# YichengDWu/tinyedm

Measured on AMD Instinct MI355X. Metric: train imgs/sec CIFAR-10 32x32 bf16, higher is better.
Workload: dtype bf16

## Files before the change

include/tinyedm_hip.h:

```cpp
#ifndef TINYEDM_HIP_H
#define TINYEDM_HIP_H
#ifdef __cplusplus
extern "C" {
#endif

typedef struct ihipStream_t* edm_stream_t;

int edm_version(void);
const char* edm_last_error(void);
int edm_init(int device);
int edm_graph_replay_safe(void);
typedef struct {
  unsigned step, seed_lo, seed_hi, reserved;
  float lr, ema_beta, grad_scale, bc1, bc2sqrt, pad[3];
} edm_step_params;

int edm_conv_igemm(const void* X, const void* Wp, void* Y, const void* R, float alpha, float beta, int B, int H,
                   int W, int Cin, int Cout, int taps, edm_stream_t stream);
int edm_conv_igemm_v2(const void* X, const void* Wp, void* Y, const void* R, float alpha, float beta, int B, int H,
                      int W, int Cin, int Cout, int taps, edm_stream_t stream);
int edm_conv_igemm_v6(const void* X, const void* Wp, void* Y, const void* R, float alpha, float beta, int B, int H,
                      int W, int Cin, int Cout, int taps, edm_stream_t stream);
int edm_conv_igemm_s(const void* X, const void* Wp, void* Y, const void* R, float alpha, float beta, int B, int H,
                     int W, int Cin, int Cout, int taps, edm_stream_t stream);
// ... 103 lines not shown
int edm_dropout_mask(unsigned char* mask, long n, float pdrop, unsigned long long seed, unsigned sub, unsigned step,
                     edm_stream_t stream);
int edm_pool2(const void* x, void* y, int B, int Hout, int Wout, int C, float scale, edm_stream_t stream);
int edm_up2(const void* x, const void* add, void* y, int B, int Hout, int Wout, int C, float scale, edm_stream_t stream);
int edm_up2_silu(const void* x, void* y, void* a, int B, int Hout, int Wout, int C, edm_stream_t stream);
int edm_reduce_hw(const void* x, long x_stride, const void* y, long y_stride, float* out, int B, int HW, int C,
                  float scale, edm_stream_t stream);
int edm_scalelong_fwd(const float* mean, const float* W1h, const float* W2h, float* gate, float* z1save, int B, int C,
                      int R, edm_stream_t stream);
int edm_scalelong_bwd(const float* mean, const float* W1h, const float* W2h, const float* gate, const float* z1save,
                      const float* ggate, float* gmean, float* gW1h, float* gW2h, int B, int C, int R,
                      edm_stream_t stream);
int edm_skip_gate_fwd(const void* skip, const float* W1h, const float* W2h, float* mean, float* gate, float* z1save,
                      int B, int HW, int C, int R, edm_stream_t stream);
int edm_skip_gate_bwd(const void* gcat, long gcat_stride, int c_off, const void* skip, const float* mean,
                      const float* W1h, const float* W2h, const float* gate, const float* z1save, float* gmean,
                      float* gW1h, float* gW2h, float* ws, int B, int HW, int C, int R, edm_stream_t stream);
typedef struct {
  const float* ws;
  const float* mean;
  float* gW1h;
  float* gW2h;
  int B, C, R, pad;
} edm_skip_gate_wgrad_item;
long edm_skip_gate_wgrad_multi_table_bytes(void);
int edm_skip_gate_wgrad_multi(const edm_skip_gate_wgrad_item* items, int n, void* table_host, void* table_dev,
                              int defer_upload, edm_stream_t stream);
typedef struct {
  const void* skip;
  const float* W1h;
  const float* W2h;
  float* mean;
  float* gate;
  float* z1save;
  void* cat;
  void* silu_out;
  int B, HW, C, R, Ci, pad;
} edm_skip_gate_fwd_item;
long edm_skip_gate_fwd_multi_table_bytes(void);
int edm_skip_gate_fwd_multi(const edm_skip_gate_fwd_item* items, int n, void* table_host, void* table_dev, int defer_upload,
                            edm_stream_t stream);
typedef struct {
  const void* gcat;
  long gcat_stride;
  const void* skip;
  const float* W1h;
  const float* W2h;
  const float* gate;
  const float* z1save;
  float* gmean;
  float* ws;
  void* gskip;
  int c_off, B, HW, C, R, pad;
} edm_skip_gate_bwd_item;
typedef struct {
  const void* gcs;
  const float* gate;
  const float* gmean;
  void* gskip;
  int B, HW, Cs, pad;
} edm_skip_half_bwd_item;
long edm_skip_gate_bwd_multi_table_bytes(void);
int edm_skip_gate_bwd_multi(const edm_skip_gate_bwd_item* items, int n, void* table_host, void* table_dev, int defer_upload,
                            edm_stream_t stream);
int edm_skip_half_bwd_multi(const edm_skip_half_bwd_item* items, int n, void* table_host, void* table_dev, int defer_upload,
                            edm_stream_t stream);
int edm_concat_gate_fwd(const void* inp, const void* skip, const float* gate, void* cat, void* silu_out, int B, int HW,
                        int Ci, int Cs, edm_stream_t stream);
int edm_concat_gate_bwd(const void* gcat, const float* gate, const float* gmean, void* ginp, void* gskip, int B,
                        int HW, int Ci, int Cs, edm_stream_t stream);
int edm_skip_half_fwd(const void* skip, const float* gate, void* cat, void* silu_out, int B, int HW, int Ci, int Cs,
                      edm_stream_t stream);
int edm_skip_half_bwd(const void* gcs, const float* gate, const float* gmean, void* gskip, int B, int HW, int Cs,
                      edm_stream_t stream);

int edm_precond_in(const float* noisy, const float* sigma, int sigma_stride, float sigma_data, void* out, int B,
                   int Cimg, int HW, int CP, edm_stream_t stream);
int edm_conv_out_fwd(const void* x, const float* w_hat, const float* gain_out, const float* noisy, const float* sigma,
                     int sigma_stride, float sigma_data, float* D, float* Fraw, int B, int HW, int C, int Co,
                     edm_stream_t stream);
int edm_conv_out_bwd(const void* x, const float* w_hat, const float* gain_out, const float* Fraw, const float* dD,
                     const float* sigma, int sigma_stride, float sigma_data, void* gx, float* gw_hat, float* ggain,
                     int B, int HW, int C, int Co, edm_stream_t stream);
int edm_nchw_to_nhwc_bf16(const float* x, void* y, int B, int C, int HW, edm_stream_t stream);
int edm_nhwc_bf16_to_nchw(const void* x, float* y, int B, int C, int HW, edm_stream_t stream);

int edm_linear_fwd(const float* X, const float* W, float* Y, int M, int N, int K, edm_stream_t stream);
int edm_linear_dgrad(const float* dY, const float* W, float* dX, int M, int N, int K, int accumulate,
                     edm_stream_t stream);
int edm_linear_wgrad(const float* dY, const float* X, float* dW, int M, int N, int K, int accumulate,
                     edm_stream_t stream);
int edm_fourier_fwd(const float* sigma, int sigma_stride, const float* freqs, const float* phases, float* out, int B,
                    int Fd, edm_stream_t stream);
int edm_embed_combine_fwd(const float* emb_sigma, const float* wcls_hat, const long long* labels, float add_factor,
                          int K, float* pre, float* out, int B, int E, edm_stream_t stream);
int edm_embed_combine_bwd(const float* gout, const float* pre, const long long* labels, float add_factor, int K,
                          float* gemb_sigma, float* gwcls_hat, int B, int E, edm_stream_t stream);

int edm_diffuse(const float* clean, float* noisy, float* sigma, float P_mean, float P_std, int B, long CHW,
                unsigned long long seed, unsigned step, const void* dyn, edm_stream_t stream);
int edm_diffuse_given(const float* clean, const float* eps, const float* noise, float* noisy, float* sigma,
                      float P_mean, float P_std, int B, long CHW, edm_stream_t stream);
int edm_weighted_mse(const float* D, const float* clean, const float* sigma, const float* weight_override,
                     float sigma_data, float* loss, float* dD, int B, long CHW, float* acc_sum, long long* acc_total,
                     edm_stream_t stream);
int edm_adam_ema(float* theta, float* grad, float* m, float* v, float* ema, long n, float lr, float b1, float b2,
                 float eps, int step, float ema_beta, float grad_scale, const void* dyn, int zero_grad,
                 unsigned* health, edm_stream_t stream);
int edm_heun_euler(const float* x, const float* D, float t0, float t1, float* dx, float* x1, long n, unsigned* health,
                   edm_stream_t stream);
int edm_heun_correct(const float* x, const float* dx, const float* x1, const float* D1, float t0, float t1, float* out,
                     long n, unsigned* health, edm_stream_t stream);
int edm_heun_euler_guided(const float* x, const float* Dm, const float* Dg, const float* w, float t0, float t1,
                          float* dx, float* x1, long n, unsigned* health, edm_stream_t stream);
int edm_heun_correct_guided(const float* x, const float* dx, const float* x1, const float* Dm1, const float* Dg1,
                            const float* w, float t0, float t1, float* out, long n, unsigned* health,
                            edm_stream_t stream);
int edm_heun_churn(const float* x, float c, const void* rec, int step, int B, long CHW, float* x_hat,
                   unsigned* health, edm_stream_t stream);
int edm_scale_f32(const float* x, float s, float* y, long n, edm_stream_t stream);

int edm_f32_conv(const float* X, const float* w_hat, float* Y, const float* R, float alpha, float beta, const float* lin,
                 long lin_stride, const float* gain, int B, int H, int W, int Cin, int I, int Cout, int taps,
                 edm_stream_t stream);
int edm_f32_to_pairs(const float* x, void* pairs, long rows, int C, edm_stream_t stream);
int edm_split_pack(const float* w_hat, void* pack, int O, int I, int taps, int Ip, edm_stream_t stream);
int edm_split_conv(const void* Xp, const void* Wp3, float* Y, void* Ypairs, const float* R, float alpha, float beta,
                   const float* lin, long lin_stride, const float* gain, int B, int H, int W, int C, int Cout, int taps,
                   edm_stream_t stream);
int edm_split_conv_o(const void* Xp, const void* Wp3, float* Y, void* Ypairs, long ld_pairs, long lo_off, void* Ysilu_pairs,
                     const float* R, float alpha, float beta, const float* lin, long lin_stride, const float* gain, int B,
                     int H, int W, int C, int Cout, int taps, edm_stream_t stream);
int edm_split_conv_fold(const void* Xp, const void* Wp3, const void* X2p, const void* W2p3, int C2, float* Y, void* Ypairs,
                        long ld_pairs, long lo_off, void* Ysilu_pairs, float alpha3, float alpha1, int B, int H, int W, int C,
                        int Cout, edm_stream_t stream);
int edm_f32_skip_half(const float* skip, const float* gate, void* cat_pairs, void* silu_pairs, int B, int HW, int Ci, int Cs,
                      edm_stream_t stream);
int edm_f32_attention(const float* qkv, float* y, int B, int N, int C, int heads, edm_stream_t stream);
int edm_split_attention(const float* qkv, float* y, void* ypairs, int B, int N, int C, int heads, edm_stream_t stream);
int edm_f32_pixelnorm_silu(const float* x, float* xn, float* s, long P, int C, int s_pairs, edm_stream_t stream);
int edm_f32_silu(const float* x, float* s, long n, int pairs_row, edm_stream_t stream);
int edm_f32_pool2(const float* x, float* y, int B, int Hout, int Wout, int C, edm_stream_t stream);
int edm_f32_up2(const float* x, float* y, int B, int Hout, int Wout, int C, edm_stream_t stream);
int edm_f32_pool_pixelnorm_silu(const float* x, float* xn, float* s, int B, int Hout, int Wout, int C, int s_pairs,
                                edm_stream_t stream);
int edm_f32_up2_silu(const float* x, float* y, float* s, int B, int Hout, int Wout, int C, int s_pairs, edm_stream_t stream);
int edm_f32_skip_gate(const float* skip, const float* W1h, const float* W2h, float* gate, int B, int HW, int C, int R,
                      edm_stream_t stream);
int edm_f32_concat_gate(const float* inp, const float* skip, const float* gate, float* cat, float* silu_out, int B,
                        int HW, int Ci, int Cs, int pairs, edm_stream_t stream);
int edm_f32_precond_in(const float* noisy, const float* sigma, int sigma_stride, float sigma_data, float* out, int B,
                       int Cimg, int HW, int CP, edm_stream_t stream);
int edm_f32_conv_out(const float* x, const float* w_hat, const float* gain_out, const float* noisy, const float* sigma,
                     int sigma_stride, float sigma_data, float* D, int B, int HW, int C, int Co, edm_stream_t stream);
int edm_f32_nchw_to_nhwc(const float* x, float* y, int B, int C, int HW, edm_stream_t stream);
int edm_f32_nhwc_to_nchw(const float* x, float* y, int B, int C, int HW, edm_stream_t stream);

int edm_u8_gather_normalize(const void* data, const long* index, float* out, int B, int C, int H, int W, long n_images,
                            float mean, float stdv, int flip, unsigned long long seed, unsigned epoch,
                            edm_stream_t stream);
int edm_denormalize_u8(const float* x, void* out, long n, float scale, float offset, edm_stream_t stream);
int edm_prediction_to_u8_nhwc(const float* pred, void* out, int B, int C, int H, int W, const float* mean,
                              const float* stdv, edm_stream_t stream);

#ifdef __cplusplus
}
// ... 3 lines not shown
```

tinyedm_amd/_lib.py:

```python
import ctypes
import os

_HERE = os.path.dirname(os.path.abspath(__file__))
LIB_PATH = os.environ.get("EDM_LIB_PATH") or os.path.join(_HERE, "libtinyedm_hip.so")

P, I, L, F = ctypes.c_void_p, ctypes.c_int, ctypes.c_long, ctypes.c_float
U, U64 = ctypes.c_uint, ctypes.c_ulonglong

SIGNATURES = {
    "edm_version": [],
    "edm_last_error": [],
    "edm_init": [I],
    "edm_graph_replay_safe": [],
    "edm_pixelnorm_silu_fwd": [P, P, P, P, L, I, P],
    "edm_pixelnorm_silu_bwd": [P, P, P, F, P, P, P, L, I, P],
    "edm_pool_pixelnorm_silu_fwd": [P, P, P, P, I, I, I, I, P],
    "edm_pool_pixelnorm_silu_bwd": [P, P, P, F, P, P, P, I, I, I, I, P],
    "edm_up2_silu": [P, P, P, I, I, I, I, P],
    "edm_silu_fwd": [P, P, L, P],
    "edm_silu_bwd": [P, P, P, F, P, L, P],
    "edm_axpby": [P, F, P, F, P, L, P],
    "edm_mod_silu_drop_fwd": [P, P, L, P, P, I, I, I, F, U64, U, U, P, P],
    "edm_mod_silu_drop_bwd": [P, P, L, P, P, P, P, P, L, P, I, I, I, F, U64, U, U, P, P],
    "edm_mod_silu_drop_bwd_raw": [P, P, L, P, P, P, P, L, I, I, I, F, U64, U, U, P, P],
    "edm_dropout_mask": [P, L, F, U64, U, U, P],
    "edm_pool2": [P, P, I, I, I, I, F, P],
    "edm_up2": [P, P, P, I, I, I, I, F, P],
    "edm_reduce_hw": [P, L, P, L, P, I, I, I, F, P],
    "edm_scalelong_fwd": [P, P, P, P, P, I, I, I, P],
    "edm_scalelong_bwd": [P, P, P, P, P, P, P, P, P, I, I, I, P],
    "edm_skip_gate_fwd": [P, P, P, P, P, P, I, I, I, I, P],
    "edm_skip_gate_bwd": [P, L, I, P, P, P, P, P, P, P, P, P, P, I, I, I, I, P],
    "edm_skip_gate_wgrad_multi": [P, I, P, P, I, P],
    "edm_skip_gate_wgrad_multi_table_bytes": [],
    "edm_skip_gate_fwd_multi": [P, I, P, P, I, P],
    "edm_skip_gate_fwd_multi_table_bytes": [],
    "edm_skip_gate_bwd_multi": [P, I, P, P, I, P],
    "edm_skip_half_bwd_multi": [P, I, P, P, I, P],
    "edm_skip_gate_bwd_multi_table_bytes": [],
    "edm_concat_gate_fwd": [P, P, P, P, P, I, I, I, I, P],
    "edm_concat_gate_bwd": [P, P, P, P, P, I, I, I, I, P],
    "edm_skip_half_fwd": [P, P, P, P, I, I, I, I, P],
    "edm_skip_half_bwd": [P, P, P, P, I, I, I, P],
    "edm_precond_in": [P, P, I, F, P, I, I, I, I, P],
    "edm_conv_out_fwd": [P, P, P, P, P, I, F, P, P, I, I, I, I, P],
    "edm_conv_out_bwd": [P, P, P, P, P, P, I, F, P, P, P, I, I, I, I, P],
    "edm_nchw_to_nhwc_bf16": [P, P, I, I, I, P],
    "edm_nhwc_bf16_to_nchw": [P, P, I, I, I, P],
    "edm_conv_igemm": [P, P, P, P, F, F, I, I, I, I, I, I, P],
    "edm_conv_igemm_v2": [P, P, P, P, F, F, I, I, I, I, I, I, P],
    "edm_conv_igemm_o": [P, P, P, L, P, P, L, I, P, F, F, I, I, I, I, I, I, I, I, P],
    "edm_conv3x3_fold_supported": [I, I, I, I, I, I],
    "edm_conv3x3_fold": [P, P, P, L, P, I, P, L, P, F, F, I, I, I, I, I, P],
    "edm_conv_igemm_v6": [P, P, P, P, F, F, I, I, I, I, I, I, P],
    "edm_conv_igemm_s": [P, P, P, P, F, F, I, I, I, I, I, I, P],
    "edm_conv3x3_mod": [P, P, P, P, P, L, P, F, U64, U, U, I, I, I, I, I, I, P, I, P],
    "edm_conv3x3_modbwd": [P, P, F, P, P, L, P, P, P, L, F, U64, U, U, I, I, I, I, I, I, P, I, P],
    "edm_mod_finish_multi": [P, P, P, L, P, I, I, P],
    "edm_conv3x3_silubwd": [P, P, P, P, F, P, I, I, I, I, I, I, P],
    "edm_mod_finish": [P, P, L, P, P, L, P, I, I, P],
    "edm_conv_wgrad_nsplit": [I, I, I, I, I, I],
    "edm_conv_wgrad_v2": [P, P, P, I, I, I, I, I, I, I, P],
    "edm_conv_wgrad_1x1_nsplit": [L, I, I],
    "edm_conv_wgrad_1x1_nsplit_grouped": [L, I, I],
    "edm_conv_wgrad_1x1": [P, P, P, L, I, I, I, P],
    "edm_conv_wgrad_1x1_group": [P, I, P, P, I, P],
    "edm_conv_wgrad_1x1_group_table_bytes": [],
    "edm_wgrad3_workspace": [P, I],
    "edm_wgrad3_group": [P, I, P, L, P, P, I, P],
    "edm_wgrad3_table_bytes": [],
    "edm_wgrad3_max_layers": [],
    "edm_attention_fwd": [P, P, I, I, I, I, P],
    "edm_attention_bwd": [P, P, P, P, I, I, I, I, P],
    "edm_attention_qkv_supported": [I, I, I],
    "edm_attention_qkv_fwd": [P, P, P, P, I, I, I, I, I, P],
    "edm_attention_qkv_bwd": [P, P, P, P, P, P, P, F, I, I, I, I, I, P],
    "edm_linear_fwd": [P, P, P, I, I, I, P],
    "edm_linear_dgrad": [P, P, P, I, I, I, I, P],
    "edm_linear_wgrad": [P, P, P, I, I, I, I, P],
    "edm_fourier_fwd": [P, I, P, P, P, I, I, P],
    "edm_embed_combine_fwd": [P, P, P, F, I, P, P, I, I, P],
    "edm_embed_combine_bwd": [P, P, P, F, I, P, P, I, I, P],
    "edm_diffuse": [P, P, P, F, F, I, L, U64, U, P, P],
    "edm_diffuse_given": [P, P, P, P, P, F, F, I, L, P],
    "edm_weighted_mse": [P, P, P, P, F, P, P, I, L, P, P, P],
    "edm_adam_ema": [P, P, P, P, P, L, F, F, F, F, I, F, F, P, I, P, P],
    "edm_heun_euler": [P, P, F, F, P, P, L, P, P],
    "edm_heun_correct": [P, P, P, P, F, F, P, L, P, P],
    "edm_heun_euler_guided": [P, P, P, P, F, F, P, P, L, P, P],
    "edm_heun_correct_guided": [P, P, P, P, P, P, F, F, P, L, P, P],
    "edm_heun_churn": [P, F, P, I, I, L, P, P, P],
    "edm_scale_f32": [P, F, P, L, P],
    "edm_weight_prep": [P, I, I, I, I, P, P, P, P, I, P],
    "edm_weight_prep_multi": [P, P, I, I, I, P],
    "edm_wgrad_finish": [P, I, P, P, P, I, I, I, I, F, I, P],
    "edm_wgrad_finish_multi": [P, I, P, P, I, P],
    "edm_wgrad_finish_multi_table_bytes": [],
    "edm_f32_conv": [P, P, P, P, F, F, P, L, P, I, I, I, I, I, I, I, P],
    "edm_f32_attention": [P, P, I, I, I, I, P],
    "edm_split_attention": [P, P, P, I, I, I, I, P],
    "edm_f32_to_pairs": [P, P, L, I, P],
    "edm_split_pack": [P, P, I, I, I, I, P],
    "edm_split_conv": [P, P, P, P, P, F, F, P, L, P, I, I, I, I, I, I, P],
    "edm_split_conv_o": [P, P, P, P, L, L, P, P, F, F, P, L, P, I, I, I, I, I, I, P],
    "edm_split_conv_fold": [P, P, P, P, I, P, P, L, L, P, F, F, I, I, I, I, I, P],
    "edm_f32_skip_half": [P, P, P, P, I, I, I, I, P],
    "edm_f32_pool_pixelnorm_silu": [P, P, P, I, I, I, I, I, P],
    "edm_f32_up2_silu": [P, P, P, I, I, I, I, I, P],
    "edm_f32_pixelnorm_silu": [P, P, P, L, I, I, P],
    "edm_f32_silu": [P, P, L, I, P],
    "edm_f32_pool2": [P, P, I, I, I, I, P],
    "edm_f32_up2": [P, P, I, I, I, I, P],
    "edm_f32_skip_gate": [P, P, P, P, I, I, I, I, P],
    "edm_f32_concat_gate": [P, P, P, P, P, I, I, I, I, I, P],
    "edm_f32_precond_in": [P, P, I, F, P, I, I, I, I, P],
    "edm_f32_conv_out": [P, P, P, P, P, I, F, P, I, I, I, I, P],
    "edm_f32_nchw_to_nhwc": [P, P, I, I, I, P],
    "edm_f32_nhwc_to_nchw": [P, P, I, I, I, P],
    "edm_u8_gather_normalize": [P, P, P, I, I, I, I, L, F, F, I, U64, U, P],
    "edm_denormalize_u8": [P, P, L, F, F, P],
    "edm_prediction_to_u8_nhwc": [P, P, I, I, I, I, P, P, P],
}
DIAG_SIGNATURES = {
    "edm_conv_igemm_v2_stamp": [P, P, P, I, I, I, I, I, P, P],
    "edm_conv_igemm_v2_ablate": [P, P, P, I, I, I, I, I, I, P],
    "edm_wgrad3_probe": [P, P],
    "edm_wgrad3_plan_ksplit": [P, I, P],
    "edm_v6_persistent_launches": [],
}
_RET = {"edm_last_error": ctypes.c_char_p, "edm_v6_persistent_launches": ctypes.c_long, "edm_wgrad3_workspace": ctypes.c_long, "edm_wgrad3_table_bytes": ctypes.c_long,
        "edm_skip_gate_wgrad_multi_table_bytes": ctypes.c_long, "edm_skip_gate_fwd_multi_table_bytes": ctypes.c_long, "edm_skip_gate_bwd_multi_table_bytes": ctypes.c_long,
        "edm_conv_wgrad_1x1_group_table_bytes": ctypes.c_long, "edm_wgrad_finish_multi_table_bytes": ctypes.c_long}
_NO_STATUS = {"edm_skip_gate_bwd_multi_table_bytes", "edm_skip_gate_fwd_multi_table_bytes", "edm_v6_persistent_launches", "edm_conv3x3_fold_supported", "edm_skip_gate_wgrad_multi_table_bytes", "edm_version", "edm_graph_replay_safe", "edm_last_error", "edm_conv_wgrad_nsplit", "edm_conv_wgrad_1x1_nsplit", "edm_conv_wgrad_1x1_nsplit_grouped", "edm_wgrad3_workspace", "edm_wgrad3_table_bytes", "edm_wgrad3_max_layers",
              "edm_conv_wgrad_1x1_group_table_bytes", "edm_wgrad_finish_multi_table_bytes", "edm_attention_qkv_supported"}

_lib = None


class HipKernelError(RuntimeError):
    pass


class FinishItem(ctypes.Structure):
    _fields_ = [("slabs", P), ("w", P), ("grad", P), ("perm", P), ("S", I), ("O", I), ("I", I), ("Ipad", I), ("taps", I),
                ("scale", F), ("accumulate", I)]


class SkipGateWgradItem(ctypes.Structure):
    _fields_ = [("ws", P), ("mean", P), ("gW1h", P), ("gW2h", P), ("B", I), ("C", I), ("R", I), ("pad", I)]


class SkipGateFwdItem(ctypes.Structure):
    _fields_ = [("skip", P), ("W1h", P), ("W2h", P), ("mean", P), ("gate", P), ("z1save", P), ("cat", P), ("silu_out", P),
                ("B", I), ("HW", I), ("C", I), ("R", I), ("Ci", I), ("pad", I)]


class SkipGateBwdItem(ctypes.Structure):
    _fields_ = [("gcat", P), ("gcat_stride", L), ("skip", P), ("W1h", P), ("W2h", P), ("gate", P), ("z1save", P), ("gmean", P),
                ("ws", P), ("gskip", P), ("c_off", I), ("B", I), ("HW", I), ("C", I), ("R", I), ("pad", I)]


class SkipHalfBwdItem(ctypes.Structure):
    _fields_ = [("gcs", P), ("gate", P), ("gmean", P), ("gskip", P), ("B", I), ("HW", I), ("Cs", I), ("pad", I)]


class WGrad1Item(ctypes.Structure):
    _fields_ = [("X", P), ("dY", P), ("slabs", P), ("npix", L), ("Cin", I), ("Cout", I), ("nsplit", I), ("pad", I)]


class WGrad3Item(ctypes.Structure):
    _fields_ = [("X", P), ("dY", P), ("w", P), ("grad", P), ("perm", P), ("B", I), ("H", I), ("W", I), ("Cin", I),
                ("Cout", I), ("I", I), ("scale", F), ("accumulate", I)]


def lib() -> ctypes.CDLL:
    global _lib
    if _lib is None:
        if not os.path.exists(LIB_PATH):
            raise RuntimeError(
                f"tinyedm_amd: {LIB_PATH} is missing -- build it with `python -m tinyedm_amd.build` "
                "(there is no CPU fallback for the HIP hot path)")
        h = ctypes.CDLL(LIB_PATH)
        for name, args in {**SIGNATURES, **DIAG_SIGNATURES}.items():
            fn = getattr(h, name)
            fn.argtypes = args
            fn.restype = _RET.get(name, ctypes.c_int)
        _lib = h
    return _lib


N_CALLS = 0


def call(name: str, *args):
    global N_CALLS
    N_CALLS += 1
    h = lib()
    rc = getattr(h, name)(*args)
    if name in _NO_STATUS:
        return rc
    if rc != 0:
        msg = h.edm_last_error()
        raise HipKernelError(f"{name} failed (status {rc}): {msg.decode() if msg else '?'}")
    return rc


_inited_devices = set()


def init_device(index: int) -> None:
    if index not in _inited_devices:
        call("edm_init", int(index))
        _inited_devices.add(index)
```

tinyedm_amd/csrc/elementwise.hip:

```cpp
#include "common.h"
#include <stdarg.h>
#include <stdio.h>

static thread_local char g_err[512] = "";
extern "C" void edm_set_error(const char* fmt, ...) {
  va_list ap;
  va_start(ap, fmt);
  vsnprintf(g_err, sizeof(g_err), fmt, ap);
  va_end(ap);
}
extern "C" const char* edm_last_error() { return g_err; }
extern "C" int edm_version() { return 1; }

static inline int cdiv(long a, long b) { return (int)((a + b - 1) / b); }
static inline int grid_for(long work, int block, int cap = 256 * 16) {
  long g = (work + block - 1) / block;
  if (g > cap) g = cap;
  if (g < 1) g = 1;
  return (int)g;
}

template <int LPP, bool POOL = false>
__global__ __launch_bounds__(256) void k_pnorm_silu_fwd(const bf16* __restrict__ x, bf16* __restrict__ xn,
                                                          bf16* __restrict__ a, float* __restrict__ dsave, int P,
// ... 1460 lines not shown
  {
    const float s = sigma[(p < pend ? b : 0) * sstride];
    cout = s * sd * rsqrtf(s * s + sd * sd);
  }
  float vn[8] = {0, 0, 0, 0, 0, 0, 0, 0}, dn[8] = {0, 0, 0, 0, 0, 0, 0, 0}, fn[8] = {0, 0, 0, 0, 0, 0, 0, 0};
  auto fetch = [&](int pp, int bb, int hh) {
    load8(x + (long)pp * C + c8 * 8, vn);
#pragma unroll
    for (int o = 0; o < 8; ++o)
      if (o < Co) {
        const long idx = ((long)bb * Co + o) * HW + hh;
        dn[o] = dD[idx];
        if (c8 == 0) fn[o] = Fraw[idx];
      }
  };
  if (p < pend) fetch(p, b, hw);
  while (p < pend) {
    float v[8], dd[8], ff[8];
#pragma unroll
    for (int j = 0; j < 8; ++j) { v[j] = vn[j]; dd[j] = dn[j]; ff[j] = fn[j]; }
    const float cur = cout;
    p += PS;
    hw += PS;
    if (hw >= HW) {
      do {
        hw -= HW;
        ++b;
      } while (hw >= HW);
      if (p < pend) {
        const float s = sigma[b * sstride];
        cout = s * sd * rsqrtf(s * s + sd * sd);
      }
    }
    if (p < pend) fetch(p, b, hw);
#pragma unroll
    for (int o = 0; o < 8; ++o) {
      if (o < Co) {
        float d = dd[o] * cur;
        if (c8 == 0) gg += d * ff[o];
        d *= go;
#pragma unroll
        for (int j = 0; j < 8; ++j) acc[o][j] += d * v[j];
      }
    }
  }
#pragma unroll
  for (int o = 0; o < 8; ++o)
    if (o < Co) {
#pragma unroll
      for (int j = 0; j < 8; ++j) red[(ps * Co + o) * C + c8 * 8 + j] = acc[o][j];
    }
  __syncthreads();
  for (int e = threadIdx.x; e < Co * C; e += blockDim.x) {
    float sacc = 0.f;
    for (int q = 0; q < PS; ++q) sacc += red[q * Co * C + e];
    atomicAdd(gwh + e, sacc);
  }
  if (c8 == 0) atomicAdd(ggain, gg);
}
extern "C" int edm_conv_out_bwd(const void* x, const float* w_hat, const float* gain_out, const float* Fraw,
                                const float* dD, const float* sigma, int sigma_stride, float sigma_data, void* gx,
                                float* gw_hat, float* ggain, int B, int HW, int C, int Co, hipStream_t st) {
  EDM_REQUIRE(B > 0 && HW > 0 && C % 8 == 0 && Co >= 1 && Co <= 8 && (sigma_stride == 0 || sigma_stride == 1),
              "conv_out_bwd: bad args");
  long npix = (long)B * HW, n8 = npix * C / 8;
  EDM_REQUIRE(n8 < (1L << 31), "conv_out_bwd: too many elements (32-bit index arithmetic)");
  hipLaunchKernelGGL(k_conv_out_bwd_x, dim3(grid_for(n8, 256)), dim3(256), 0, st, dD, w_hat, gain_out, sigma,
                     sigma_stride, sigma_data, (bf16*)gx, HW, C, Co, n8);
  EDM_CHECK_LAUNCH("conv_out_bwd_x");
  {
    const int CL = C / 8;
    EDM_REQUIRE(CL <= 256, "conv_out_bwd: C=%d too large", C);
    int block = (256 / CL) * CL, PS = block / CL;
    while (PS > 1 && (size_t)PS * Co * C * sizeof(float) > 48 * 1024) { --PS; block = PS * CL; }
    const int PIXW = 256;
    hipLaunchKernelGGL(k_conv_out_bwd_w, dim3(cdiv(npix, PIXW)), dim3(block), (size_t)PS * Co * C * sizeof(float), st,
                       (const bf16*)x, dD, Fraw, gain_out, sigma, sigma_stride, sigma_data, gw_hat, ggain, HW, C, Co,
                       npix, PIXW);
  }
  EDM_CHECK_LAUNCH("conv_out_bwd_w");
  return EDM_OK;
}

__global__ void k_nchw_f32_to_nhwc_bf16(const float* __restrict__ x, bf16* __restrict__ y, int C, int HW, long n8) {
  const int CL = C >> 3;
  for (long i = (long)blockIdx.x * blockDim.x + threadIdx.x; i < n8; i += (long)gridDim.x * blockDim.x) {
    int c8 = (int)(i % CL);
    long p = i / CL;
    long b = p / HW;
    int hw = (int)(p % HW);
    float v[8];
#pragma unroll
    for (int j = 0; j < 8; ++j) v[j] = x[(b * C + c8 * 8 + j) * HW + hw];
    store8(y + i * 8, v);
  }
}
__global__ void k_nhwc_bf16_to_nchw_f32(const bf16* __restrict__ x, float* __restrict__ y, int C, int HW, long n8) {
  const int CL = C >> 3;
  for (long i = (long)blockIdx.x * blockDim.x + threadIdx.x; i < n8; i += (long)gridDim.x * blockDim.x) {
    int c8 = (int)(i % CL);
    long p = i / CL;
    long b = p / HW;
    int hw = (int)(p % HW);
    float v[8];
    load8(x + i * 8, v);
#pragma unroll
    for (int j = 0; j < 8; ++j) y[(b * C + c8 * 8 + j) * HW + hw] = v[j];
  }
}
extern "C" int edm_nchw_to_nhwc_bf16(const float* x, void* y, int B, int C, int HW, hipStream_t st) {
  EDM_REQUIRE(B > 0 && C % 8 == 0 && HW > 0, "nchw_to_nhwc_bf16: bad args");
  long n8 = (long)B * HW * C / 8;
  hipLaunchKernelGGL(k_nchw_f32_to_nhwc_bf16, dim3(grid_for(n8, 256)), dim3(256), 0, st, x, (bf16*)y, C, HW, n8);
  EDM_CHECK_LAUNCH("nchw_to_nhwc_bf16");
  return EDM_OK;
}
extern "C" int edm_nhwc_bf16_to_nchw(const void* x, float* y, int B, int C, int HW, hipStream_t st) {
  EDM_REQUIRE(B > 0 && C % 8 == 0 && HW > 0, "nhwc_bf16_to_nchw: bad args");
  long n8 = (long)B * HW * C / 8;
  hipLaunchKernelGGL(k_nhwc_bf16_to_nchw_f32, dim3(grid_for(n8, 256)), dim3(256), 0, st, (const bf16*)x, y, C, HW, n8);
  EDM_CHECK_LAUNCH("nhwc_bf16_to_nchw");
  return EDM_OK;
}
```

tinyedm_amd/ops.py:

```python
import ctypes
import math
import os
from typing import Optional

import torch

from . import _lib

bf16, f32 = torch.bfloat16, torch.float32

PROFILE = None


class _prof:
    def __init__(self, name, flops, nbytes):
        self.name, self.flops, self.nbytes = name, flops, nbytes

    def __enter__(self):
        if PROFILE is not None:
            self.s = torch.cuda.Event(enable_timing=True)
            self.e = torch.cuda.Event(enable_timing=True)
            self.s.record()
        return self

# ... 556 lines not shown

def skip_gate_wgrad_multi(items):
    n = len(items)
    if not 0 < n <= 32:
        raise ValueError("skip_gate_wgrad_multi: 1..32 gates per launch")
    arr = (_lib.SkipGateWgradItem * n)()
    out = []
    for k, (ws, mean, R) in enumerate(items):
        _chk(mean, f32, "mean")
        B, C = mean.shape
        _chk(ws, f32, "ws", (B, C + 2 * R))
        gw1 = torch.empty(R, C + 1, device=ws.device, dtype=f32)
        gw2 = torch.empty(C, R, device=ws.device, dtype=f32)
        arr[k] = _lib.SkipGateWgradItem(ws.data_ptr(), mean.data_ptr(), gw1.data_ptr(), gw2.data_ptr(), B, C, R, 0)
        out.append((gw1, gw2))
    th, td, defer, release = _tables.take(items[0][0].device)
    _lib.call("edm_skip_gate_wgrad_multi", ctypes.byref(arr), n, ctypes.c_void_p(th), ctypes.c_void_p(td), defer, _stream())
    release()
    return out


def concat_gate_fwd(inp, skip, gate, want_silu):
    B, H, W, Ci = _nhwc(inp, "inp")
    Bs, Hs, Ws, Cs = _nhwc(skip, "skip")
    if (Bs, Hs, Ws) != (B, H, W):
        raise ValueError("concat_gate_fwd: inp/skip spatial mismatch")
    _chk(gate, f32, "gate", (B, Cs))
    cat = torch.empty(B, H, W, Ci + Cs, device=inp.device, dtype=bf16)
    sil = torch.empty_like(cat) if want_silu else None
    _lib.call("edm_concat_gate_fwd", _p(inp), _p(skip), _p(gate), _p(cat), _p(sil), B, H * W, Ci, Cs, _stream())
    return cat, sil


def concat_gate_bwd(gcat, gate, gmean, Ci):
    B, H, W, Ct = _nhwc(gcat, "gcat")
    Cs = Ct - Ci
    _chk(gate, f32, "gate", (B, Cs))
    _chk(gmean, f32, "gmean", (B, Cs))
    ginp = torch.empty(B, H, W, Ci, device=gcat.device, dtype=bf16)
    gskip = torch.empty(B, H, W, Cs, device=gcat.device, dtype=bf16)
    _lib.call("edm_concat_gate_bwd", _p(gcat), _p(gate), _p(gmean), _p(ginp), _p(gskip), B, H * W, Ci, Cs, _stream())
    return ginp, gskip


def skip_half_fwd(skip, gate, cat, sil=None):
    B, H, W, Cs = _nhwc(skip, "skip")
    _chk(gate, f32, "gate", (B, Cs))
    Ct = cat.shape[-1]
    _chk(cat, bf16, "cat", (B, H, W, Ct))
    if sil is not None:
        _chk(sil, bf16, "sil", (B, H, W, Ct))
    if Ct <= Cs:
        raise ValueError("skip_half_fwd: cat must be wider than the skip")
    _lib.call("edm_skip_half_fwd", _p(skip), _p(gate), _p(cat), _p(sil), B, H * W, Ct - Cs, Cs, _stream())


def skip_half_bwd(gcs, gate, gmean):
    B, H, W, Cs = _nhwc(gcs, "gcs")
    _chk(gate, f32, "gate", (B, Cs))
    _chk(gmean, f32, "gmean", (B, Cs))
    gskip = torch.empty_like(gcs)
    _lib.call("edm_skip_half_bwd", _p(gcs), _p(gate), _p(gmean), _p(gskip), B, H * W, Cs, _stream())
    return gskip


def _sigma_arg(sigma, B):
    _chk(sigma, f32, "sigma")
    if sigma.numel() == 1:
        return 0
    if sigma.numel() != B:
        raise ValueError(f"sigma must have 1 or {B} elements, got {sigma.numel()}")
    return 1


def precond_in(noisy, sigma, sigma_data, CP):
    _chk(noisy, f32, "noisy")
    B, Cimg, H, W = noisy.shape
    ss = _sigma_arg(sigma, B)
    out = torch.empty(B, H, W, CP, device=noisy.device, dtype=bf16)
    _lib.call("edm_precond_in", _p(noisy), _p(sigma), ss, float(sigma_data), _p(out), B, Cimg, H * W, CP, _stream())
    return out


def conv_out_fwd(x, w_hat, gain_out, noisy, sigma, sigma_data, want_fraw=True):
    B, H, W, C = _nhwc(x, "x")
    Co = w_hat.shape[0]
    _chk(w_hat, f32, "w_hat", (Co, C))
    _chk(noisy, f32, "noisy", (B, Co, H, W))
    _chk(gain_out, f32, "gain_out")
    ss = _sigma_arg(sigma, B)
    D = torch.empty(B, Co, H, W, device=x.device, dtype=f32)
    Fraw = torch.empty(B, Co, H, W, device=x.device, dtype=f32) if want_fraw else None
    _lib.call("edm_conv_out_fwd", _p(x), _p(w_hat), _p(gain_out), _p(noisy), _p(sigma), ss, float(sigma_data), _p(D),
              _p(Fraw), B, H * W, C, Co, _stream())
    return D, Fraw


def conv_out_bwd(x, w_hat, gain_out, Fraw, dD, sigma, sigma_data, gg_out=None):
    B, H, W, C = _nhwc(x, "x")
    Co = w_hat.shape[0]
    _chk(dD, f32, "dD", (B, Co, H, W))
    _chk(Fraw, f32, "Fraw", (B, Co, H, W))
    ss = _sigma_arg(sigma, B)
    gx = torch.empty_like(x)
    gw = zeros_f32(w_hat.shape, w_hat.device)
    gg = zeros_f32((), x.device) if gg_out is None else _chk(gg_out, f32, "gg_out", ())
    _lib.call("edm_conv_out_bwd", _p(x), _p(w_hat), _p(gain_out), _p(Fraw), _p(dD), _p(sigma), ss, float(sigma_data),
              _p(gx), _p(gw), _p(gg), B, H * W, C, Co, _stream())
    return gx, gw, gg


def nchw_to_nhwc_bf16(x):
    _chk(x, f32, "x")
    B, C, H, W = x.shape
    y = torch.empty(B, H, W, C, device=x.device, dtype=bf16)
    _lib.call("edm_nchw_to_nhwc_bf16", _p(x), _p(y), B, C, H * W, _stream())
    return y


def nhwc_bf16_to_nchw(x):
    B, H, W, C = _nhwc(x, "x")
    y = torch.empty(B, C, H, W, device=x.device, dtype=f32)
    _lib.call("edm_nhwc_bf16_to_nchw", _p(x), _p(y), B, C, H * W, _stream())
    return y


IGEMM_VERSION = int(os.environ.get("EDM_IGEMM", "0"))


def _igemm_entry(npix, W, Cout, taps, Cin=0):
    if taps == 9 and W > 64:
        return "edm_conv_igemm"
    if IGEMM_VERSION == 1:
        return "edm_conv_igemm"
    if IGEMM_VERSION == 2:
        return "edm_conv_igemm_v2"
    if IGEMM_VERSION == 6:
        ok = taps == 9 and Cin % 64 == 0 and Cin <= 2016 and W <= 64
        return "edm_conv_igemm_v6" if ok else "edm_conv_igemm"
    if IGEMM_VERSION == 5:
        return "edm_conv_igemm_s" if (taps == 9 and Cin % 256 == 0 and Cin <= 2016 and W <= 16) else "edm_conv_igemm"
    if taps == 9:
        tm = (npix + 511) // 512
        tiles3 = tm * ((Cout + 127) // 128)
        v6_ok = Cin % 64 == 0 and Cin <= 2016 and W <= 64
        if tiles3 >= 512:
            return "edm_conv_igemm_v6" if v6_ok else "edm_conv_igemm"
        if v6_ok and tm * ((Cout + 63) // 64) >= 256:
            return "edm_conv_igemm_v6"
        ts = ((npix + 127) // 128) * ((Cout + 63) // 64)
        if W <= 16 and Cin % 256 == 0 and Cin <= 2016 and 128 <= ts <= 1024:
            return "edm_conv_igemm_s"
        return "edm_conv_igemm"
    tiles2 = ((npix + 255) // 256) * ((Cout + 127) // 128)
    return "edm_conv_igemm_v2" if tiles2 >= 1024 else "edm_conv_igemm"


def uses_s_kernel(npix, W, Cin, Cout):
    return (IGEMM_VERSION == 0 and Cout % 64 == 0 and Cin % 32 == 0
            and _igemm_entry(npix, W, Cout, 9, Cin) == "edm_conv_igemm_s")


def _wfrag(wp, entry, who):
    if not getattr(wp, "_edm_frag", False):
        return 0
    if entry != "edm_conv_igemm_s":
        raise ValueError(f"{who}: a fragment-major weight pack reached a shape that does not run on k_conv3x3_s ({entry})")
    return 1


V46 = "_v6"
_KERNEL_ID = {"edm_conv_igemm": 1, "edm_conv_igemm_v2": 2, "edm_conv_igemm_s": 5, "edm_conv_igemm_v6": 6}


def _v4_suffix(entry, npix, Cout):
    if entry == "edm_conv_igemm_s":
        return "_s"
    if entry != "edm_conv_igemm_v6":
        return entry[len("edm_conv_igemm"):]
    pad4, pad2 = (Cout + 127) // 128 * 128, (Cout + 63) // 64 * 64
    wide = ((npix + 511) // 512) * ((Cout + 127) // 128) >= 512 and not pad2 * 80 < pad4 * 69
    return V46 if wide else V46 + "s"


def conv_igemm(x, wp, taps, residual=None, alpha=1.0, beta=0.0, out=None, silu_out=None, split=None):
    B, H, W, Cin = _nhwc(x, "x")
    _chk(wp, bf16, "wp")
    if wp.dim() != 3 or wp.shape[0] != taps or wp.shape[2] != Cin:
        raise ValueError(f"conv_igemm: packed weight {tuple(wp.shape)} does not match taps={taps}, Cin={Cin}")
    Cout = wp.shape[1]
    if residual is not None:
# ... 954 lines not shown
```

Measured before the change: 10230.

## Use MFMA for output conv forward and fused slab-reduced backward

Adds a forward output-projection kernel that runs the 1x1 conv on MFMA bf16 instructions. The fp32 weights are split into three bf16 parts (high, mid, low) so the result keeps roughly fp32 precision. Adds a fused backward kernel that computes the input gradient, per-block weight-gradient slabs and the gain gradient in one pass, followed by a deterministic slab-sum kernel. This replaces the atomics or zero-initialised accumulation of the old path. Both are enabled by default through EDM_NET_ENDS; the cost is a workspace allocation per call and an extra launch.

After: 10260 (median of 6 runs). About the same (+0.3%).

```diff
diff --git a/include/tinyedm_hip.h b/include/tinyedm_hip.h
--- a/include/tinyedm_hip.h
+++ b/include/tinyedm_hip.h
@@ -209,6 +209,13 @@
 int edm_conv_out_bwd(const void* x, const float* w_hat, const float* gain_out, const float* Fraw, const float* dD,
                      const float* sigma, int sigma_stride, float sigma_data, void* gx, float* gw_hat, float* ggain,
                      int B, int HW, int C, int Co, edm_stream_t stream);
+int edm_conv_out_fwd2(const void* x, const float* w_hat, const float* gain_out, const float* noisy, const float* sigma,
+                      int sigma_stride, float sigma_data, float* D, float* Fraw, int B, int HW, int C, int Co,
+                      edm_stream_t stream);
+long edm_conv_out_bwd2_workspace(int B, int HW, int C, int Co);
+int edm_conv_out_bwd2(const void* x, const float* w_hat, const float* gain_out, const float* Fraw, const float* dD,
+                      const float* sigma, int sigma_stride, float sigma_data, void* gx, float* gw_hat, float* ggain,
+                      void* workspace, long workspace_bytes, int B, int HW, int C, int Co, edm_stream_t stream);
 int edm_nchw_to_nhwc_bf16(const float* x, void* y, int B, int C, int HW, edm_stream_t stream);
 int edm_nhwc_bf16_to_nchw(const void* x, float* y, int B, int C, int HW, edm_stream_t stream);
 
diff --git a/tinyedm_amd/_lib.py b/tinyedm_amd/_lib.py
--- a/tinyedm_amd/_lib.py
+++ b/tinyedm_amd/_lib.py
@@ -45,6 +45,9 @@
     "edm_precond_in": [P, P, I, F, P, I, I, I, I, P],
     "edm_conv_out_fwd": [P, P, P, P, P, I, F, P, P, I, I, I, I, P],
     "edm_conv_out_bwd": [P, P, P, P, P, P, I, F, P, P, P, I, I, I, I, P],
+    "edm_conv_out_fwd2": [P, P, P, P, P, I, F, P, P, I, I, I, I, P],
+    "edm_conv_out_bwd2_workspace": [I, I, I, I],
+    "edm_conv_out_bwd2": [P, P, P, P, P, P, I, F, P, P, P, P, L, I, I, I, I, P],
     "edm_nchw_to_nhwc_bf16": [P, P, I, I, I, P],
     "edm_nhwc_bf16_to_nchw": [P, P, I, I, I, P],
     "edm_conv_igemm": [P, P, P, P, F, F, I, I, I, I, I, I, P],
@@ -128,10 +131,10 @@
     "edm_wgrad3_plan_ksplit": [P, I, P],
     "edm_v6_persistent_launches": [],
 }
-_RET = {"edm_last_error": ctypes.c_char_p, "edm_v6_persistent_launches": ctypes.c_long, "edm_wgrad3_workspace": ctypes.c_long, "edm_wgrad3_table_bytes": ctypes.c_long,
+_RET = {"edm_last_error": ctypes.c_char_p, "edm_conv_out_bwd2_workspace": ctypes.c_long, "edm_v6_persistent_launches": ctypes.c_long, "edm_wgrad3_workspace": ctypes.c_long, "edm_wgrad3_table_bytes": ctypes.c_long,
         "edm_skip_gate_wgrad_multi_table_bytes": ctypes.c_long, "edm_skip_gate_fwd_multi_table_bytes": ctypes.c_long, "edm_skip_gate_bwd_multi_table_bytes": ctypes.c_long,
         "edm_conv_wgrad_1x1_group_table_bytes": ctypes.c_long, "edm_wgrad_finish_multi_table_bytes": ctypes.c_long}
-_NO_STATUS = {"edm_skip_gate_bwd_multi_table_bytes", "edm_skip_gate_fwd_multi_table_bytes", "edm_v6_persistent_launches", "edm_conv3x3_fold_supported", "edm_skip_gate_wgrad_multi_table_bytes", "edm_version", "edm_graph_replay_safe", "edm_last_error", "edm_conv_wgrad_nsplit", "edm_conv_wgrad_1x1_nsplit", "edm_conv_wgrad_1x1_nsplit_grouped", "edm_wgrad3_workspace", "edm_wgrad3_table_bytes", "edm_wgrad3_max_layers",
+_NO_STATUS = {"edm_conv_out_bwd2_workspace", "edm_skip_gate_bwd_multi_table_bytes", "edm_skip_gate_fwd_multi_table_bytes", "edm_v6_persistent_launches", "edm_conv3x3_fold_supported", "edm_skip_gate_wgrad_multi_table_bytes", "edm_version", "edm_graph_replay_safe", "edm_last_error", "edm_conv_wgrad_nsplit", "edm_conv_wgrad_1x1_nsplit", "edm_conv_wgrad_1x1_nsplit_grouped", "edm_wgrad3_workspace", "edm_wgrad3_table_bytes", "edm_wgrad3_max_layers",
               "edm_conv_wgrad_1x1_group_table_bytes", "edm_wgrad_finish_multi_table_bytes", "edm_attention_qkv_supported"}
 
 _lib = None
diff --git a/tinyedm_amd/csrc/elementwise.hip b/tinyedm_amd/csrc/elementwise.hip
--- a/tinyedm_amd/csrc/elementwise.hip
+++ b/tinyedm_amd/csrc/elementwise.hip
@@ -1566,6 +1566,248 @@
   return EDM_OK;
 }
 
+__global__ __launch_bounds__(256) void k_conv_out_fwd_mfma(const bf16* __restrict__ x, const float* __restrict__ wh,
+                                                           const float* __restrict__ gain_out,
+                                                           const float* __restrict__ noisy,
+                                                           const float* __restrict__ sigma, int sstride, float sd,
+                                                           float* __restrict__ D, float* __restrict__ Fraw, int HW, int C,
+                                                           int Co, int npix) {
+  extern __shared__ __attribute__((aligned(16))) bf16x8 wfrag[];
+  const int lane = threadIdx.x & 63, wave = threadIdx.x >> 6;
+  const int nkb = (C + 31) >> 5, CL = C >> 3;
+  for (int i = threadIdx.x; i < nkb * 64; i += blockDim.x) {
+    const int kb = i >> 6, l = i & 63, n = l & 15, k0 = kb * 32 + 8 * (l >> 4);
+    bf16x8 h, m, lo;
+#pragma unroll
+    for (int j = 0; j < 8; ++j) {
+      const float w = (n < Co && k0 + j < C) ? wh[(long)n * C + k0 + j] : 0.f;
+      const bf16 wh0 = (bf16)w;
+      const float r1 = w - (float)wh0;
+      const bf16 wm = (bf16)r1;
+      h[j] = wh0;
+      m[j] = wm;
+      lo[j] = (bf16)(r1 - (float)wm);
+    }
+    wfrag[(kb * 3 + 0) * 64 + l] = h;
+    wfrag[(kb * 3 + 1) * 64 + l] = m;
+    wfrag[(kb * 3 + 2) * 64 + l] = lo;
+  }
+  __syncthreads();
+  const float go = *gain_out;
+  const int ntiles = (npix + 15) >> 4, row = lane & 15, kq = lane >> 4;
+  const bf16x8 zero8 = {};
+  for (int t = blockIdx.x * 4 + wave; t < ntiles; t += gridDim.x * 4) {
+    const bf16* xr = x + (long)min(t * 16 + row, npix - 1) * C;
+    f32x4 acc = {0.f, 0.f, 0.f, 0.f};
+    constexpr int KU = 8;
+    for (int kb0 = 0; kb0 < nkb; kb0 += KU) {
+      bf16x8 a[KU];
+#pragma unroll
+      for (int u = 0; u < KU; ++u) {
+        const int c8 = (kb0 + u) * 4 + kq;
+        a[u] = *reinterpret_cast<const bf16x8*>(xr + 8 * min(c8, CL - 1));
+        if (c8 >= CL) a[u] = zero8;
+      }
+#pragma unroll
+      for (int u = 0; u < KU; ++u) {
+        if (kb0 + u < nkb) {
+          const bf16x8* f = wfrag + (kb0 + u) * 3 * 64 + lane;
+          acc = __builtin_amdgcn_mfma_f32_16x16x32_bf16(a[u], f[0], acc, 0, 0, 0);
+          acc = __builtin_amdgcn_mfma_f32_16x16x32_bf16(a[u], f[64], acc, 0, 0, 0);
+          acc = __builtin_amdgcn_mfma_f32_16x16x32_bf16(a[u], f[128], acc, 0, 0, 0);
+        }
+      }
+    }
+    const int o = lane & 15;
+    if (o < Co) {
+#pragma unroll
+      for (int r = 0; r < 4; ++r) {
+        const int p = t * 16 + 4 * kq + r;
+        if (p < npix) {
+          const int b = p / HW, hw = p - b * HW;
+          const float s = sigma[b * sstride];
+          const float den = s * s + sd * sd;
+          const float cskip = sd * sd / den, cout = s * sd * rsqrtf(den);
+          const long idx = ((long)b * Co + o) * HW + hw;
+          if (Fraw) Fraw[idx] = acc[r];
+          D[idx] = acc[r] * go * cout + noisy[idx] * cskip;
+        }
+      }
+    }
+  }
+}
+extern "C" int edm_conv_out_fwd2(const void* x, const float* w_hat, const float* gain_out, const float* noisy,
+                                 const float* sigma, int sigma_stride, float sigma_data, float* D, float* Fraw, int B,
+                                 int HW, int C, int Co, hipStream_t st) {
+  EDM_REQUIRE(B > 0 && HW > 0 && C % 8 == 0 && C > 0 && C <= 1024 && Co >= 1 && Co <= 16 &&
+                  (sigma_stride == 0 || sigma_stride == 1),
+              "conv_out_fwd2: bad args (C <= 1024, Co <= 16 required)");
+  const long npix = (long)B * HW;
+  EDM_REQUIRE(npix + 16 < (1L << 31) && npix * C < (1L << 40), "conv_out_fwd2: too many pixels");
+  const int lds = ((C + 31) / 32) * 3 * 64 * 16;
+  EDM_MAX_LDS(k_conv_out_fwd_mfma, 96 * 1024);
+  const long tiles = (npix + 15) / 16;
+  const int grid = (int)(tiles < 4096 ? (tiles + 3) / 4 : 1024);
+  hipLaunchKernelGGL(k_conv_out_fwd_mfma, dim3(grid), dim3(256), lds, st, (const bf16*)x, w_hat, gain_out, noisy, sigma,
+                     sigma_stride, sigma_data, D, Fraw, HW, C, Co, (int)npix);
+  EDM_CHECK_LAUNCH("conv_out_fwd2");
+  return EDM_OK;
+}
+
+template <int CO>
+__global__ __launch_bounds__(256) void k_conv_out_bwd_fused(const bf16* __restrict__ x, const float* __restrict__ dD,
+                                                            const float* __restrict__ Fraw,
+                                                            const float* __restrict__ wh,
+                                                            const float* __restrict__ gain_out,
+                                                            const float* __restrict__ sigma, int sstride, float sd,
+                                                            bf16* __restrict__ gx, float* __restrict__ slabs, int HW,
+                                                            int C, int Co, int npix, int PIXW) {
+  extern __shared__ __attribute__((aligned(16))) float red[];
+  constexpr int U = 4;
+  const int CL = C >> 3;
+  const int PS = blockDim.x / CL;
+  const int c8 = threadIdx.x % CL, ps = threadIdx.x / CL;
+  const int p0 = blockIdx.x * PIXW, p1 = min(npix, p0 + PIXW);
+  const float go = *gain_out;
+  float w[CO][8], acc[CO][8];
+#pragma unroll
+  for (int o = 0; o < CO; ++o)
+#pragma unroll
+    for (int j = 0; j < 8; ++j) {
+      w[o][j] = o < Co ? wh[(long)o * C + c8 * 8 + j] : 0.f;
+      acc[o][j] = 0.f;
+    }
+  float gg = 0.f;
+  for (int pb = p0 + ps; pb < p1; pb += U * PS) {
+    float v[U][8], dd[U][CO], ff[U][CO], co[U];
+#pragma unroll
+    for (int u = 0; u < U; ++u) {
+      const int p = pb + u * PS;
+      const bool ok = p < p1;
+      const int b = ok ? p / HW : 0, hw = ok ? p - b * HW : 0;
+      if (ok) load8(x + (long)p * C + c8 * 8, v[u]);
+      else
+#pragma unroll
+        for (int j = 0; j < 8; ++j) v[u][j] = 0.f;
+      const float s = sigma[b * sstride];
+      co[u] = ok ? s * sd * rsqrtf(s * s + sd * sd) : 0.f;
+#pragma unroll
+      for (int o = 0; o < CO; ++o) {
+        const long idx = ((long)b * Co + o) * HW + hw;
+        dd[u][o] = (ok && o < Co) ? dD[idx] : 0.f;
+        ff[u][o] = (ok && o < Co && c8 == 0) ? Fraw[idx] : 0.f;
+      }
+    }
+#pragma unroll
+    for (int u = 0; u < U; ++u) {
+      float g[8] = {0, 0, 0, 0, 0, 0, 0, 0};
+#pragma unroll
+      for (int o = 0; o < CO; ++o) {
+        float d = dd[u][o] * co[u];
+        gg += d * ff[u][o];
+        d *= go;
+#pragma unroll
+        for (int j = 0; j < 8; ++j) {
+          g[j] += d * w[o][j];
+          acc[o][j] += d * v[u][j];
+        }
+      }
+      const int p = pb + u * PS;
+      if (p < p1) store8(gx + (long)p * C + c8 * 8, g);
+    }
+  }
+  const int CC = Co * C;
+#pragma unroll
+  for (int o = 0; o < CO; ++o)
+    if (o < Co) {
+#pragma unroll
+      for (int j = 0; j < 8; ++j) red[(ps * Co + o) * C + c8 * 8 + j] = acc[o][j];
+    }
+  if (c8 == 0) red[PS * CC + ps] = gg;
+  __syncthreads();
+  float* slab = slabs + (long)blockIdx.x * (CC + 1);
+  for (int e = threadIdx.x; e < CC; e += blockDim.x) {
+    float sacc = 0.f;
+    for (int q = 0; q < PS; ++q) sacc += red[q * CC + e];
+    slab[e] = sacc;
+  }
+  if (threadIdx.x == 0) {
+    float sacc = 0.f;
+    for (int q = 0; q < PS; ++q) sacc += red[PS * CC + q];
+    slab[CC] = sacc;
+  }
+}
+__global__ __launch_bounds__(256) void k_conv_out_bwd_sum(const float* __restrict__ slabs, int G, int CC,
+                                                          float* __restrict__ gwh, float* __restrict__ ggain) {
+  __shared__ float part[16][16];
+  const int c = threadIdx.x & 15, q = threadIdx.x >> 4, col = blockIdx.x * 16 + c;
+  float s[4] = {0.f, 0.f, 0.f, 0.f};
+  if (col <= CC) {
+    int g = q;
+    for (; g + 48 < G; g += 64) {
+#pragma unroll
+      for (int k = 0; k < 4; ++k) s[k] += slabs[(long)(g + 16 * k) * (CC + 1) + col];
+    }
+    for (int k = 0; g < G; g += 16, ++k) s[k] += slabs[(long)g * (CC + 1) + col];
+  }
+  part[q][c] = (s[0] + s[1]) + (s[2] + s[3]);
+  __syncthreads();
+  if (q == 0 && col <= CC) {
+    float t = 0.f;
+    for (int k = 0; k < 16; ++k) t += part[k][c];
+    if (col < CC) gwh[col] = t;
+    else *ggain += t;
+  }
+}
+namespace {
+constexpr int CO_BWD_PIXW = 256;
+int conv_out_bwd_split(int C, int Co, int* block) {
+  const int CL = C / 8;
+  int PS = 256 / CL;
+  while (PS > 1 && ((size_t)PS * Co * C + PS) * sizeof(float) > 64 * 1024) --PS;
+  *block = PS * CL;
+  return PS;
+}
+}
+extern "C" long edm_conv_out_bwd2_workspace(int B, int HW, int C, int Co) {
+  if (B <= 0 || HW <= 0 || C <= 0 || Co <= 0) return -1;
+  const long G = ((long)B * HW + CO_BWD_PIXW - 1) / CO_BWD_PIXW;
+  return G * ((long)Co * C + 1) * (long)sizeof(float);
+}
+extern "C" int edm_conv_out_bwd2(const void* x, const float* w_hat, const float* gain_out, const float* Fraw,
+                                 const float* dD, const float* sigma, int sigma_stride, float sigma_data, void* gx,
+                                 float* gw_hat, float* ggain, void* workspace, long workspace_bytes, int B, int HW, int C,
+                                 int Co, hipStream_t st) {
+  EDM_REQUIRE(B > 0 && HW > 0 && C % 8 == 0 && C > 0 && C <= 1024 && Co >= 1 && Co <= 8 &&
+                  (sigma_stride == 0 || sigma_stride == 1),
+              "conv_out_bwd2: bad args (C <= 1024, Co <= 8 required)");
+  const long npix = (long)B * HW;
+  EDM_REQUIRE(npix + 256L * CO_BWD_PIXW < (1L << 31), "conv_out_bwd2: too many pixels (32-bit index arithmetic)");
+  const long need = edm_conv_out_bwd2_workspace(B, HW, C, Co);
+  EDM_REQUIRE(workspace && workspace_bytes >= need, "conv_out_bwd2: workspace too small (%ld < %ld bytes)",
+              workspace_bytes, need);
+  int block = 0;
+  const int PS = conv_out_bwd_split(C, Co, &block);
+  const size_t lds = ((size_t)PS * Co * C + PS) * sizeof(float);
+  const int G = (int)((npix + CO_BWD_PIXW - 1) / CO_BWD_PIXW);
+  float* slabs = (float*)workspace;
+  if (Co <= 4) {
+    EDM_MAX_LDS(k_conv_out_bwd_fused<4>, 64 * 1024);
+    hipLaunchKernelGGL(k_conv_out_bwd_fused<4>, dim3(G), dim3(block), lds, st, (const bf16*)x, dD, Fraw, w_hat, gain_out,
+                       sigma, sigma_stride, sigma_data, (bf16*)gx, slabs, HW, C, Co, (int)npix, CO_BWD_PIXW);
+  } else {
+    EDM_MAX_LDS(k_conv_out_bwd_fused<8>, 64 * 1024);
+    hipLaunchKernelGGL(k_conv_out_bwd_fused<8>, dim3(G), dim3(block), lds, st, (const bf16*)x, dD, Fraw, w_hat, gain_out,
+                       sigma, sigma_stride, sigma_data, (bf16*)gx, slabs, HW, C, Co, (int)npix, CO_BWD_PIXW);
+  }
+  EDM_CHECK_LAUNCH("conv_out_bwd2");
+  const int CC = Co * C;
+  hipLaunchKernelGGL(k_conv_out_bwd_sum, dim3((CC + 1 + 15) / 16), dim3(256), 0, st, (const float*)slabs, G, CC, gw_hat,
+                     ggain);
+  EDM_CHECK_LAUNCH("conv_out_bwd_sum");
+  return EDM_OK;
+}
+
 __global__ void k_nchw_f32_to_nhwc_bf16(const float* __restrict__ x, bf16* __restrict__ y, int C, int HW, long n8) {
   const int CL = C >> 3;
   for (long i = (long)blockIdx.x * blockDim.x + threadIdx.x; i < n8; i += (long)gridDim.x * blockDim.x) {
diff --git a/tinyedm_amd/ops.py b/tinyedm_amd/ops.py
--- a/tinyedm_amd/ops.py
+++ b/tinyedm_amd/ops.py
@@ -662,6 +662,9 @@
     return out
 
 
+NET_ENDS = os.environ.get("EDM_NET_ENDS", "1") != "0"
+
+
 def conv_out_fwd(x, w_hat, gain_out, noisy, sigma, sigma_data, want_fraw=True):
     B, H, W, C = _nhwc(x, "x")
     Co = w_hat.shape[0]
@@ -671,8 +674,8 @@
     ss = _sigma_arg(sigma, B)
     D = torch.empty(B, Co, H, W, device=x.device, dtype=f32)
     Fraw = torch.empty(B, Co, H, W, device=x.device, dtype=f32) if want_fraw else None
-    _lib.call("edm_conv_out_fwd", _p(x), _p(w_hat), _p(gain_out), _p(noisy), _p(sigma), ss, float(sigma_data), _p(D),
-              _p(Fraw), B, H * W, C, Co, _stream())
+    _lib.call("edm_conv_out_fwd2" if NET_ENDS else "edm_conv_out_fwd", _p(x), _p(w_hat), _p(gain_out), _p(noisy),
+              _p(sigma), ss, float(sigma_data), _p(D), _p(Fraw), B, H * W, C, Co, _stream())
     return D, Fraw
 
 
@@ -683,10 +686,19 @@
     _chk(Fraw, f32, "Fraw", (B, Co, H, W))
     ss = _sigma_arg(sigma, B)
     gx = torch.empty_like(x)
-    gw = zeros_f32(w_hat.shape, w_hat.device)
     gg = zeros_f32((), x.device) if gg_out is None else _chk(gg_out, f32, "gg_out", ())
-    _lib.call("edm_conv_out_bwd", _p(x), _p(w_hat), _p(gain_out), _p(Fraw), _p(dD), _p(sigma), ss, float(sigma_data),
-              _p(gx), _p(gw), _p(gg), B, H * W, C, Co, _stream())
+    if not NET_ENDS:
+        gw = zeros_f32(w_hat.shape, w_hat.device)
+        _lib.call("edm_conv_out_bwd", _p(x), _p(w_hat), _p(gain_out), _p(Fraw), _p(dD), _p(sigma), ss,
+                  float(sigma_data), _p(gx), _p(gw), _p(gg), B, H * W, C, Co, _stream())
+        return gx, gw, gg
+    gw = torch.empty(w_hat.shape, device=w_hat.device, dtype=f32)
+    nb = _lib.lib().edm_conv_out_bwd2_workspace(B, H * W, C, Co)
+    if nb <= 0:
+        raise ValueError(f"conv_out_bwd: bad shape B={B} HW={H * W} C={C} Co={Co}")
+    work = torch.empty(nb // 4, device=x.device, dtype=f32)
+    _lib.call("edm_conv_out_bwd2", _p(x), _p(w_hat), _p(gain_out), _p(Fraw), _p(dD), _p(sigma), ss, float(sigma_data),
+              _p(gx), _p(gw), _p(gg), _p(work), nb, B, H * W, C, Co, _stream())
     return gx, gw, gg
 
 
```
